# cold-deuu/Quadrotor_Manipulator_MPPI

Hardware: AMD Instinct MI355X
Metric: MPPI rollouts/sec (K x H state-steps) + control-step p50 latency, K=4096 H=32 (higher is better)
Workload: dtype f32

## Files before the change

### quadrotor_manipulator_mppi_amd/csrc/mppi_finalize.hip

```cpp
#include <algorithm>

#include "mppi_device.h"

using namespace mppi;

constexpr int kFinThreads = 512;
constexpr int kMaxRec = 4096;
#ifndef MPPI_FIN_KO
#define MPPI_FIN_KO 0
#endif
#ifndef MPPI_FIN_NOMARK
#define MPPI_FIN_NOMARK 0
#endif
#ifndef MPPI_FIN_XCDS
#define MPPI_FIN_XCDS 8
#endif

#if defined(MPPI_STAMPS) && !defined(MPPI_TIMELINE)
#define FSTAMP(i)                                                                    \
    do {                                                                             \
        __builtin_amdgcn_sched_barrier(0);                                           \
        if (pk.stamps && threadIdx.x == 0)                                           \
            pk.stamps[(((size_t)v * A + a) * ts + sl) * kStamps + (i)] =               \
                __builtin_amdgcn_s_memtime();                                        \
        __builtin_amdgcn_sched_barrier(0);                                           \
    } while (0)
#define FSTAMPRT(i) do { } while (0)
#elif defined(MPPI_STAMPS)
#define FSTAMPRT(i)                                                                  \
    do {                                                                             \
        if (pk.stamps && threadIdx.x == 0) {                                         \
            pk.stamps[(((size_t)v * A + a) * ts + sl) * kStamps + (i)] =               \
                __builtin_amdgcn_s_memrealtime();                                    \
            if ((i) == 13)                                                           \
                pk.stamps[(((size_t)v * A + a) * ts + sl) * kStamps + 15] =            \
                    (unsigned long long)__builtin_amdgcn_s_getreg(0xF814);           \
        }                                                                            \
    } while (0)
#define FSTAMP(i) do { if ((i) == 1 || (i) == 7) FSTAMPRT(i); } while (0)
#else
#define FSTAMP(i) do { } while (0)
#define FSTAMPRT(i) do { } while (0)
#endif

enum { kRoleAny = 0, kRoleFinal = 1, kRoleQuiet = 2, kRolePack = 3, kRolePeer = 4 };
struct GeoRt { static constexpr bool kStatic = false; static constexpr int A = 0, H = 0, tsz = 0, hf = 0, ts = 0; };
template <int A_, int H_, int TSZ_, int HF_, int TS_>
struct GeoC { static constexpr bool kStatic = true; static constexpr int A = A_, H = H_, tsz = TSZ_, hf = HF_, ts = TS_; };

template <int CW, int WIN, int NT, int ROLE, typename GEO>
__device__ __forceinline__ void fin_body(const float* __restrict__ hdr_base, const float* __restrict__ dat_base,
                                         const FinTail* __restrict__ tail, const uint32_t nrec_H, const uint32_t geo,
                                         const int32_t hdr_rs, const int32_t d_rs, const int32_t d_as,
                                         const int32_t hdr_vs, const int32_t d_vs, const uint32_t seq_arg,
                                         const FinParams& pk) {
    constexpr bool kAny = ROLE == kRoleAny, kQuiet = ROLE == kRoleQuiet;
    constexpr bool kOut = kAny || ROLE == kRoleFinal || ROLE == kRolePeer;
    constexpr bool kUpd = kOut || kQuiet;
    constexpr bool kPeer = kAny || ROLE == kRolePeer;
    constexpr int NWV = NT / 64;
    constexpr int ROWS = 64 / CW;
    constexpr int TR = NWV * ROWS;
    constexpr int kNPT = 16;
    __shared__ float wcol[NWV][CW];
    __shared__ float wrho[NWV], wnan[NWV], weta[NWV], weta2[NWV];
    __shared__ float wsg[96];
    const FinParams& p = pk;
    const int tid = threadIdx.x, lane = tid & 63, wv = tid >> 6;
    const int n = (int)(nrec_H & 0xFFFFu);
    const int H = GEO::kStatic ? GEO::H : (int)(nrec_H >> 16);
    const int tsz = GEO::kStatic ? GEO::tsz : (int)(geo & 0xFFu), hf = GEO::kStatic ? GEO::hf : (int)((geo >> 8) & 0xFFu);
    const int ts = GEO::kStatic ? GEO::ts : (int)((geo >> 16) & 0xFFu), A = GEO::kStatic ? GEO::A : (int)(geo >> 24);
    const int x8 = blockIdx.x & 7, j8 = blockIdx.x >> 3, na = (A + MPPI_FIN_XCDS - 1) / MPPI_FIN_XCDS;
    const int sl = (na == 1) ? j8 : (na == 2) ? (j8 >> 1) : j8 / na;
    const int a = x8 + MPPI_FIN_XCDS * (j8 - sl * na), v = blockIdx.y;
    if (x8 >= MPPI_FIN_XCDS || a >= A) return;
    if (MPPI_FIN_KO & 16) { if (tid == 0) p.u_prev[blockIdx.x] = 0.0f; return; }
    FSTAMPRT(13);
    FSTAMP(0);
    const int t_lo = sl * tsz, t_hi = min(H, t_lo + tsz);
    const int w0 = max(0, t_lo - hf), w1 = min(H, t_hi + hf), W = w1 - w0;
    const float* hdr = uniform_ptr(hdr_base + (size_t)v * (uint32_t)hdr_vs);
    const float* col = uniform_ptr(dat_base + (size_t)v * (uint32_t)d_vs + (size_t)a * d_as + w0);
    const FinTail& T = *tail;
    const int g = lane / CW, q = lane - g * CW, gr = wv * ROWS + g;
    const bool qv = q < W;
    float u_old = 0.0f, x0f = 0.0f, v0f = 0.0f;
    double x0d = 0.0, v0d = 0.0;
    float* up = nullptr;

    float coef = 0.0f, dt = 0.0f, dt2 = 0.0f;
    int32_t mode = (ROLE == kRolePack) ? 1 : 0, model = 0, qoff = 0, nq = 0, sf64 = 0, odim = 0;
    const uint32_t seq = seq_arg;
    uint32_t seqv = seq;
    float *wraw = nullptr, *wsmooth = nullptr, *u0p = nullptr, *stats = nullptr;
    double* outp = nullptr;
    uint32_t* flags = nullptr;
    const VehicleConst* vcb = nullptr;
    unsigned long long* const* xpeers = nullptr;
    unsigned long long xpl = 0ull;
    unsigned long long* xlocal = nullptr;
    uint32_t* xovl = nullptr;
    uint32_t* xstall = nullptr;
    unsigned long long* xdec = nullptr;
    int32_t xn = 0, xme = 0;
    uint32_t xstep = 0u, xep = 0u;
    float sg[WIN > 0 ? WIN : 1];
    auto pin_tail = [&]() {
        coef = T.coef;
        if constexpr (kAny) {
            dt = T.dt; dt2 = T.dt2;
            mode = T.mode; model = T.model; qoff = T.qoff; nq = T.nq; sf64 = T.state_f64; odim = T.out_dim;
            wraw = T.wraw; wsmooth = T.wsmooth; u0p = T.u0; stats = T.stats; outp = T.out; flags = T.flags;
            up = T.u_prev; vcb = T.vc;
            xpeers = T.xpeers; xlocal = T.xlocal; xn = T.xn; xme = T.xme; xovl = T.xovl; xstall = T.xstall; xdec = T.xdec;
        } else {
            if constexpr (kOut) {
                dt = T.dt; dt2 = T.dt2;
                model = T.model; qoff = T.qoff; nq = T.nq; sf64 = T.state_f64; odim = T.out_dim;
                u0p = T.u0; stats = T.stats; outp = T.out; flags = T.flags; vcb = T.vc;
            }
            if constexpr (kUpd) up = T.u_prev;
            if constexpr (ROLE == kRolePeer) {
                xpeers = T.xpeers; xlocal = T.xlocal; xn = T.xn; xme = T.xme; xstall = T.xstall; xdec = T.xdec;
            }
        }
        if constexpr (WIN > 0 && kUpd) {
#pragma unroll
            for (int j = 0; j < WIN; ++j) sg[j] = T.sg[j];
        }
        if constexpr (kAny)
            asm volatile("" : "+s"(coef), "+s"(dt), "+s"(dt2), "+s"(mode), "+s"(model), "+s"(qoff), "+s"(nq),
                              "+s"(sf64), "+s"(odim), "+s"(wraw), "+s"(wsmooth), "+s"(u0p), "+s"(stats),
                              "+s"(outp), "+s"(flags), "+s"(up), "+s"(vcb), "+s"(xpeers), "+s"(xlocal), "+s"(xn),
                              "+s"(xme), "+s"(xovl), "+s"(xstall), "+s"(xdec));
        else if constexpr (kOut) {
            asm volatile("" : "+s"(coef), "+s"(dt), "+s"(dt2), "+s"(model), "+s"(qoff), "+s"(nq), "+s"(sf64),
                              "+s"(odim), "+s"(u0p), "+s"(stats), "+s"(outp), "+s"(flags), "+s"(up), "+s"(vcb));
            if constexpr (ROLE == kRolePeer)
                asm volatile("" : "+s"(xpeers), "+s"(xlocal), "+s"(xn), "+s"(xme), "+s"(xstall), "+s"(xdec));
        } else if constexpr (kQuiet)
            asm volatile("" : "+s"(coef), "+s"(up));
        else
            asm volatile("" : "+s"(coef));
        if constexpr (WIN == 9 && kUpd)
            asm volatile("" : "+s"(sg[0]), "+s"(sg[1]), "+s"(sg[2]), "+s"(sg[3]), "+s"(sg[4]), "+s"(sg[5]),
                              "+s"(sg[6]), "+s"(sg[7]), "+s"(sg[8]));
        else if constexpr (WIN == 5 && kUpd)
            asm volatile("" : "+s"(sg[0]), "+s"(sg[1]), "+s"(sg[2]), "+s"(sg[3]), "+s"(sg[4]));
        if constexpr (kUpd) {
            up += (size_t)v * H * A;
            if (wv == 0 && q < W && g == 0) u_old = ld_dev(up + (w0 + q) * A + a);
        }
        if constexpr (kOut) {
            if (tid == 0 && sl == 0) {
                const VehicleConst* vcp = vcb + v;
                x0f = ld_dev(vcp->pos0f + a); v0f = ld_dev(vcp->vel0f + a);
                x0d = ld_dev(vcp->pos0 + a); v0d = ld_dev(vcp->vel0 + a);
                if (seq == kSeqFromVc) seqv = ld_dev((const uint32_t*)vcp->_pad);
            }
        }
        if constexpr (kPeer) {
            if (tid == 0 && xpeers) {
                xstep = ld_dev((const uint32_t*)(vcb + v) + kVcStepWord);
                xep = ld_dev((const uint32_t*)(vcb + v) + kVcEpochWord);
            }
            if (wv == 0 && xpeers)
                xpl = ((const __attribute__((address_space(1))) unsigned long long*)xpeers)[lane < xn ? lane : 0];
        }
    };
    float rho_t = INFINITY, acc = 0.0f, nanflag = 0.0f, eta = 0.0f, eta2 = 0.0f;
    const uint32_t hrs_b = (uint32_t)hdr_rs * 4u, drs_b = (uint32_t)d_rs * 4u;
    const __amdgpu_buffer_rsrc_t hrsrc =
        __builtin_amdgcn_make_buffer_rsrc(const_cast<float*>(hdr), 0, __builtin_amdgcn_readfirstlane((int)((uint32_t)n * hrs_b)),
                                          0x00020000);
    const __amdgpu_buffer_rsrc_t crsrc = __builtin_amdgcn_make_buffer_rsrc(
        const_cast<float*>(col), 0, __builtin_amdgcn_readfirstlane((int)((uint32_t)(n - 1) * drs_b + (uint32_t)W * 4u)),
        0x00020000);
    typedef uint32_t u32x4 __attribute__((ext_vector_type(4)));
    for (int base = 0; base < n; base += TR * kNPT) {
        float4 hd[kNPT];
        float xv[kNPT];
        uint32_t okm = 0;
        const uint32_t r0 = (uint32_t)(base + gr);
        const uint32_t hoff = r0 * hrs_b, coff = r0 * drs_b + (uint32_t)(qv ? q : 0) * 4u;
#pragma unroll
        for (int i = 0; i < kNPT; ++i) {
            okm |= (uint32_t)(r0 + (uint32_t)(i * TR) < (uint32_t)n) << i;
            const u32x4 h = __builtin_amdgcn_raw_buffer_load_b128(hrsrc, (int)(hoff + (uint32_t)(i * TR) * hrs_b), 0, kAuxDev);
            hd[i] = make_float4(__uint_as_float(h.x), __uint_as_float(h.y), __uint_as_float(h.z), __uint_as_float(h.w));
            xv[i] = __uint_as_float(__builtin_amdgcn_raw_buffer_load_b32(crsrc, (int)(coff + (uint32_t)(i * TR) * drs_b), 0, kAuxDev));
        }
        if (base == 0) {
            __builtin_amdgcn_sched_barrier(0);
            pin_tail();
        }
#pragma unroll
        for (int i = 0; i < kNPT; ++i)
            if (!((okm >> i) & 1u)) hd[i].x = INFINITY;
        FSTAMP(7);
        float m = INFINITY;
#pragma unroll
        for (int i = 0; i < kNPT; ++i) { m = fminf(m, hd[i].x); nanflag = fmaxf(nanflag, hd[i].w); }
        float fr[kNPT];
#pragma unroll
        for (int i = 0; i < kNPT; ++i) fr[i] = 0.0f;
        if (m < INFINITY) {
            const float rn = fminf(rho_t, m);
            if (rho_t < INFINITY) {
                const float sc = __expf(coef * (rho_t - rn));
                acc *= sc;
                eta *= sc;
                eta2 *= sc * sc;
            }
            rho_t = rn;
#pragma unroll
            for (int i = 0; i < kNPT; ++i) {
                const float f = (hd[i].x < INFINITY) ? __expf(coef * (hd[i].x - rn)) : 0.0f;
                fr[i] = f;
                eta = fmaf(f, hd[i].y, eta);
                eta2 = fmaf(f * f, hd[i].z, eta2);
            }
        }
#pragma unroll
        for (int i = 0; i < kNPT; ++i) acc = fmaf(fr[i], xv[i], acc);
        FSTAMP(8);
    }
    {
        const float rw = fold_rows<CW>(rho_t, OpMin());
        const float sc = (rho_t < INFINITY) ? __expf(coef * (rho_t - rw)) : 0.0f;
        acc = fold_rows<CW>(acc * sc, OpAdd());
        const float e1 = fold_rows<CW>(eta * sc, OpAdd()), e2 = fold_rows<CW>(eta2 * (sc * sc), OpAdd());
        const float nf = fold_rows<CW>(nanflag, OpMax());
        if (lane < CW) wcol[wv][lane] = acc;
        if (lane == 0) { wrho[wv] = rw; wnan[wv] = nf; weta[wv] = e1; weta2[wv] = e2; }
    }
    FSTAMP(1);
    if (MPPI_FIN_KO & 8) { if (lane < CW) p.u_prev[lane] += acc + (float)eta; return; }
    lds_barrier();
    if (wv != 0) return;
    FSTAMP(2);
    float rho = wrho[0], nanf = wnan[0];
#pragma unroll
    for (int w = 1; w < NWV; ++w) { rho = fminf(rho, wrho[w]); nanf = fmaxf(nanf, wnan[w]); }
    float N = 0.0f;
    eta = 0.0f; eta2 = 0.0f;
#pragma unroll
    for (int w = 0; w < NWV; ++w) {
        const float f = (wrho[w] < INFINITY) ? __expf(coef * (wrho[w] - rho)) : 0.0f;
        N = fmaf(f, (lane < CW) ? wcol[w][lane] : 0.0f, N);
        eta = fmaf(f, weta[w], eta);
        eta2 = fmaf(f * f, weta2[w], eta2);
    }
    FSTAMP(3);
    bool xlate = false;
    if (kPeer && xpeers != nullptr && mode != 1) {
        const uint32_t step = __builtin_amdgcn_readfirstlane(xstep);
        const uint32_t tag = peer_tag(step, __builtin_amdgcn_readfirstlane(xep));
        const size_t nbk = (size_t)8 * na * ts, blk = blockIdx.x;
        const size_t par = step & 1u;
        const float hown = (lane == 0) ? rho : (lane == 1) ? eta : (lane == 2) ? eta2 : nanf;
        const size_t off = ((par * (size_t)xn + (size_t)xme) * nbk + blk) * kXW;
        typedef __attribute__((address_space(1))) unsigned long long gst64;
        auto region = [&](int d) {
            return (gst64*)(((uint64_t)(uint32_t)__builtin_amdgcn_readlane((int)(uint32_t)(xpl >> 32), d) << 32) |
                            (uint32_t)__builtin_amdgcn_readlane((int)(uint32_t)xpl, d));
        };
        typedef __attribute__((address_space(1))) unsigned long long gu64;
        gu64* const ctl = (gu64*)xlocal - kXCtl;
        if (mode == 0) {
            if (uint32_t* xs = xstall) {
                const uint32_t sv = ld_dev(xs);
                if (sv != 0u && (sv & 0xFFFFu) == (uint32_t)blk) {
                    const uint64_t t_s = __builtin_amdgcn_s_memrealtime(), ticks = (uint64_t)(sv >> 16) * 100000ull;
                    while (__builtin_amdgcn_s_memrealtime() - t_s < ticks) __builtin_amdgcn_s_sleep(127);
                    if (lane == 0) __hip_atomic_store(xs, 0u, __ATOMIC_RELAXED, __HIP_MEMORY_SCOPE_AGENT);
                }
            }
            const unsigned long long wc = ((unsigned long long)tag << 32) | __float_as_uint(N);
            const unsigned long long wh = ((unsigned long long)tag << 32) | __float_as_uint(hown);
#pragma unroll
            for (int d = 0; d < kMaxPeers; ++d) {
                if (d >= xn || d == xme) continue;
                gst64* dst = region(d) + off;
                if (lane < W) __hip_atomic_store(dst + kHdr + lane, wc, __ATOMIC_RELAXED, __HIP_MEMORY_SCOPE_SYSTEM);
                if (lane < kHdr) __hip_atomic_store(dst + lane, wh, __ATOMIC_RELAXED, __HIP_MEMORY_SCOPE_SYSTEM);
            }
        }
        float nv[kMaxPeers], hv[kMaxPeers];
#pragma unroll
        for (int r = 0; r < kMaxPeers; ++r) {
            nv[r] = (r == xme) ? N : 0.0f;
            hv[r] = (r == xme) ? hown : 0.0f;
        }
        const bool needc = lane < W, needh = lane < kHdr;
        uint32_t pend = ((1u << xn) - 1u) & ~(1u << xme);
        const unsigned long long* src = xlocal + (par * (size_t)xn * nbk + blk) * kXW;
        auto poll = [&](bool heed_reports) -> bool {
            const uint64_t t_in = __builtin_amdgcn_s_memrealtime();
            while (pend != 0u) {
                unsigned long long xc[kMaxPeers], xh[kMaxPeers];
#pragma unroll
                for (int r = 0; r < kMaxPeers; ++r) {
                    xc[r] = 0ull; xh[r] = 0ull;
                    if ((pend >> r) & 1u) {
                        gu64* s = (gu64*)(src + (size_t)r * nbk * kXW);
                        xc[r] = __hip_atomic_load(s + kHdr + lane, __ATOMIC_RELAXED, __HIP_MEMORY_SCOPE_SYSTEM);
                        xh[r] = __hip_atomic_load(s + (lane & (kHdr - 1)), __ATOMIC_RELAXED, __HIP_MEMORY_SCOPE_SYSTEM);
                    }
                }
                if (heed_reports) {
                    const unsigned long long xk = __hip_atomic_load(ctl + (lane < xn ? lane : 0), __ATOMIC_RELAXED,
                                                                    __HIP_MEMORY_SCOPE_SYSTEM);
                    if (__builtin_amdgcn_ballot_w64(lane < xn && xk != 0ull) != 0ull) return true;
                }
#pragma unroll
                for (int r = 0; r < kMaxPeers; ++r) {
                    if (!((pend >> r) & 1u)) continue;
                    const bool ok = (!needc || (uint32_t)(xc[r] >> 32) == tag) && (!needh || (uint32_t)(xh[r] >> 32) == tag);
                    if (__builtin_amdgcn_ballot_w64(!ok) == 0ull) {
                        nv[r] = needc ? __uint_as_float((uint32_t)xc[r]) : 0.0f;
                        hv[r] = needh ? __uint_as_float((uint32_t)xh[r]) : 0.0f;
                        pend &= ~(1u << r);
                    }
                }
                pend = __builtin_amdgcn_readfirstlane(pend);
                if (pend == 0u) break;
                if (__builtin_amdgcn_s_memrealtime() - t_in > kPeerWaitTicks) return true;
                __builtin_amdgcn_s_sleep(1);
            }
            return false;
        };
        bool late = poll(true), torn = false;
        if (mode == 0) {
            gu64* dw = (gu64*)xdec + par * nbk;
            if (!late) {
                if (lane == 0 && !MPPI_FIN_NOMARK)
                    __hip_atomic_store(dw + blk, ((unsigned long long)tag << 32) | kDecCommit, __ATOMIC_RELAXED,
                                       __HIP_MEMORY_SCOPE_AGENT);
            } else {
                const unsigned long long cw = ((unsigned long long)tag << 32) | 1ull;
#pragma unroll
                for (int d = 0; d < kMaxPeers; ++d) {
                    if (d >= xn) continue;
                    gst64* rg = region(d);
                    if (lane == 0) __hip_atomic_store(rg - kXCtl + xme, cw, __ATOMIC_RELAXED, __HIP_MEMORY_SCOPE_SYSTEM);
                }
                const uint64_t t_rep = __builtin_amdgcn_s_memrealtime();
                while (__builtin_amdgcn_s_memrealtime() - t_rep < kDecGraceTicks) __builtin_amdgcn_s_sleep(8);
                bool marked = false;
                for (size_t i = lane; i < nbk; i += 64) {
                    const unsigned long long w = __hip_atomic_load(dw + i, __ATOMIC_RELAXED, __HIP_MEMORY_SCOPE_AGENT);
                    marked |= (uint32_t)(w >> 32) == tag && ((uint32_t)w & 3u) == kDecCommit;
                }
                if (__builtin_amdgcn_ballot_w64(marked) != 0ull) {
                    late = poll(false);
                    torn = late;
                }
                uint32_t* xe = T.xerr;
                if (late && lane == 0 && xe) {
                    __hip_atomic_store(xe, tag, __ATOMIC_RELAXED, __HIP_MEMORY_SCOPE_SYSTEM);
                    if (torn) __hip_atomic_store(xe + 1, tag, __ATOMIC_RELAXED, __HIP_MEMORY_SCOPE_SYSTEM);
                }
            }
        }
        rho = INFINITY;
        nanf = late ? (torn ? 3.0f : 2.0f) : 0.0f;
#pragma unroll
        for (int r = 0; r < kMaxPeers; ++r) {
            if (r < xn) {
                rho = fminf(rho, __int_as_float(__builtin_amdgcn_readlane(__float_as_int(hv[r]), 0)));
                nanf = fmaxf(nanf, __int_as_float(__builtin_amdgcn_readlane(__float_as_int(hv[r]), 3)));
            }
        }
        N = 0.0f; eta = 0.0f; eta2 = 0.0f;
#pragma unroll
        for (int r = 0; r < kMaxPeers; ++r) {
            if (r < xn) {
                const float rr = __int_as_float(__builtin_amdgcn_readlane(__float_as_int(hv[r]), 0));
                const float er = __int_as_float(__builtin_amdgcn_readlane(__float_as_int(hv[r]), 1));
                const float e2 = __int_as_float(__builtin_amdgcn_readlane(__float_as_int(hv[r]), 2));
                const float f = (rr < INFINITY) ? __expf(coef * (rr - rho)) : 0.0f;
                N = fmaf(f, nv[r], N);
                eta = fmaf(f, er, eta);
                eta2 = fmaf(f * f, e2, eta2);
            }
        }
        if (late) { xlate = true; N = 0.0f; }
    }
    const int t = w0 + lane;
    const bool own = lane < W && t >= t_lo && t < t_hi;
    if (mode == 1) {
        float* dst = T.dst;
        float* xbase = T.xbase;
        int64_t xslot = T.xslot;
        int32_t nslots = T.nslots, myslot = T.myslot, P = T.P;
        asm volatile("" : "+s"(dst), "+s"(xbase), "+s"(xslot), "+s"(nslots), "+s"(myslot), "+s"(P));
        dst += (size_t)v * P;
        if (a == 0 && sl == 0 && lane == 0) {
            dst[0] = rho; dst[1] = eta; dst[2] = eta2; dst[3] = nanf;
        }
        if (own) dst[kHdr + a * H + t] = N;
        for (int s = 0; s < nslots; ++s) {
            if (s == myslot) continue;
            float* z = xbase + (size_t)s * xslot + (size_t)v * P;
            if (a == 0 && sl == 0 && lane < kHdr) z[lane] = 0.0f;
            if (own) z[kHdr + a * H + t] = 0.0f;
        }
        FSTAMPRT(14);
        return;
    }

    const float etaf = xlate ? 1.0f : (nanf > 0.0f) ? NAN : eta;
    const float w = __fdividef(N, etaf);
    FSTAMP(4);
    constexpr int kPad = kMaxW / 2;
    static_assert(kPad + 64 + kMaxW / 2 <= (int)(sizeof(wsg) / sizeof(float)),
                  "wsg holds the widest window: kPad + W (<= 64) + hf");
    float sm = 0.0f;
    if (lane < W) {
        wsg[kPad + lane] = w;
        if (w0 == 0 && t < hf) wsg[kPad - 1 - t] = w;
        if (w1 == H && t >= H - hf) wsg[kPad + 2 * H - 1 - t - w0] = w;
    }
    wave_lds_handoff();
    {
        const float* src = wsg + kPad + lane - hf;
        if constexpr (WIN > 0) {
#pragma unroll
            for (int j = 0; j < WIN; ++j) sm = fmaf(sg[j], src[j], sm);
        } else {
            for (int j = 0; j < T.window; ++j) sm = fmaf(T.sg[j], src[j], sm);
        }
    }
// ... 18 lines not shown
        if (plain) u0p[(size_t)v * A + a] = u0;
        double* out = outp + (size_t)v * odim;
        const bool drone_dim = (model == MPPI_MODEL_DRONE) || (model == MPPI_MODEL_WHOLEBODY && a < 3);
        double o1 = 0.0, o2 = 0.0;
        if (model == MPPI_MODEL_QUADROTOR) {
        } else if (drone_dim) {
            const float x0 = x0f, v0 = v0f;
            const float xo = (x0 + v0 * dt) + (0.5f * u0) * dt2;
            const float vo = v0 + dt * u0;
            o1 = xo;
            o2 = vo;
            if (plain) {
                out[a] = o1;
                out[3 + a] = o2;
            }
        } else {
            const int j = a - qoff;
            const int base = (model == MPPI_MODEL_WHOLEBODY) ? 6 : 0;
            const float t1 = uold0 * dt;
            const float t2 = ((0.5f * u0) * dt) * dt;
            const float t3 = u0 * dt;
            if (sf64 && model == MPPI_MODEL_ARM) {
                o1 = (x0d + (double)t1) + (double)t2;
                o2 = v0d + (double)t3;
            } else {
                o1 = (double)((x0f + t1) + t2);
                o2 = (double)(v0f + t3);
            }
            if (plain) {
                out[base + j] = o1;
                out[base + nq + j] = o2;
            }
        }
        const float ess = (eta2 > 0.0f) ? eta * (eta / eta2) : 0.0f;
        if (plain && a == 0) {
            float* st = stats + (size_t)v * 4;
            st[0] = rho;
            st[1] = eta;
            st[2] = ess;
            st[3] = nanf;
        }
        if (seqv != 0u) {
            typedef uint32_t u32x4 __attribute__((ext_vector_type(4)));
            u32x4* rec = reinterpret_cast<u32x4*>(flags) + (size_t)v * (2 * A + 1);
            const uint64_t b1 = (uint64_t)__double_as_longlong(o1), b2 = (uint64_t)__double_as_longlong(o2);
            rec[2 * a] = u32x4{(uint32_t)b1, (uint32_t)(b1 >> 32), __float_as_uint(u0), seqv};
            rec[2 * a + 1] = u32x4{(uint32_t)b2, (uint32_t)(b2 >> 32), __float_as_uint(nanf), seqv};
            if (a == 0) rec[2 * A] = u32x4{__float_as_uint(rho), __float_as_uint(eta), __float_as_uint(ess), seqv};
        }
    }
    FSTAMP(6);
    FSTAMPRT(14);
    if (!(MPPI_FIN_KO & 128)) asm volatile("s_waitcnt vmcnt(0)" ::: "memory");
    if (xovl != nullptr && mode == 0 && lane == 0)
        __hip_atomic_fetch_add(xovl + ((size_t)v * A + a) * ts + sl, 1u, __ATOMIC_RELAXED, __HIP_MEMORY_SCOPE_AGENT);
}

template <int CW, int WIN, int NT>
__global__ void __launch_bounds__(NT) k_finalize(const float* __restrict__ hdr_base,
                                                          const float* __restrict__ dat_base,
                                                          const FinTail* __restrict__ tail,
                                                          const uint32_t nrec_H, const uint32_t geo,
                                                          const int32_t hdr_rs, const int32_t d_rs,
                                                          const int32_t d_as, const int32_t hdr_vs,
                                                          const int32_t d_vs, const uint32_t seq_arg,
                                                          const FinParams pk) {
    fin_body<CW, WIN, NT, kRoleAny, GeoRt>(hdr_base, dat_base, tail, nrec_H, geo, hdr_rs, d_rs, d_as, hdr_vs, d_vs,
                                           seq_arg, pk);
}

template <int GID> struct FinGeo;
template <> struct FinGeo<1> { typedef GeoC<7, 32, 8, 4, 4> type; static constexpr int win = 9; };
template <> struct FinGeo<2> { typedef GeoC<3, 32, 8, 2, 4> type; static constexpr int win = 5; };
template <> struct FinGeo<3> { typedef GeoC<4, 32, 8, 2, 4> type; static constexpr int win = 5; };
template <> struct FinGeo<4> { typedef GeoC<10, 64, 8, 4, 8> type; static constexpr int win = 9; };
constexpr int kFinGeoCW = 16;
static int fin_geo_id(const FinParams* p) {
    if (p->tsz != 8 || p->half != p->window / 2 || p->ts * 8 != p->H) return 0;
    if (p->window == 9) return (p->H == 32 && p->A == 7) ? 1 : (p->H == 64 && p->A == 10) ? 4 : 0;
    if (p->window == 5) return (p->H == 32 && p->A == 3) ? 2 : (p->H == 32 && p->A == 4) ? 3 : 0;
    return 0;
}

template <int NT, int ROLE, int GID>
__global__ void __launch_bounds__(NT) k_finalize_s(const float* __restrict__ hdr_base,
                                                            const float* __restrict__ dat_base,
                                                            const FinTail* __restrict__ tail,
                                                            const uint32_t nrec_H, const uint32_t geo,
                                                            const int32_t hdr_rs, const int32_t d_rs,
                                                            const int32_t d_as, const int32_t hdr_vs,
                                                            const int32_t d_vs, const uint32_t seq_arg,
                                                            const FinParams pk) {
    fin_body<kFinGeoCW, FinGeo<GID>::win, NT, ROLE, typename FinGeo<GID>::type>(hdr_base, dat_base, tail, nrec_H, geo, hdr_rs,
                                                                          d_rs, d_as, hdr_vs, d_vs, seq_arg, pk);
}

extern "C" __global__ void __launch_bounds__(64) k_dispatch_probe(unsigned long long* out) {
    if (threadIdx.x == 0) out[0] = mppi_dispatch_id();
}

extern "C" __global__ void __launch_bounds__(64) k_peer_probe(unsigned long long* const* peers,
                                                              unsigned long long* local, int n, int me,
                                                              unsigned long long slot_words, uint32_t tag,
                                                              unsigned long long ticks,
                                                              unsigned long long* out) {
    const int lane = threadIdx.x;
    const unsigned long long w = ((unsigned long long)(tag | (uint32_t)me) << 32) | 0x3F800000ull;
    if (lane < n) __hip_atomic_store(peers[lane] + (size_t)me * slot_words, w, __ATOMIC_RELAXED, __HIP_MEMORY_SCOPE_SYSTEM);
    unsigned long long got = 0ull;
    if (lane < n) {
        const uint64_t t0 = __builtin_amdgcn_s_memrealtime();
        for (;;) {
            got = __hip_atomic_load(local + (size_t)lane * slot_words, __ATOMIC_RELAXED, __HIP_MEMORY_SCOPE_SYSTEM);
            if ((uint32_t)(got >> 32) == (tag | (uint32_t)lane)) break;
            if (__builtin_amdgcn_s_memrealtime() - t0 > ticks) break;
            __builtin_amdgcn_s_sleep(2);
        }
        out[lane] = got;
    }
}

extern "C" int mppi_launch_peer_probe(unsigned long long* const* peers, unsigned long long* local, int n, int me,
                                      unsigned long long slot_words, uint32_t tag, unsigned long long ticks,
                                      unsigned long long* out, void* stream) {
    hipLaunchKernelGGL(k_peer_probe, dim3(1), dim3(64), 0, (hipStream_t)stream, peers, local, n, me, slot_words, tag,
                       ticks, out);
    return (int)hipGetLastError();
}

__global__ void k_weights(const float* S, const float* stats, float* w, int V, int K, float coef) {
    const int i = blockIdx.x * blockDim.x + threadIdx.x;
    if (i >= V * K) return;
    const int v = i / K;
    const float rho = stats[v * 4], eta = stats[v * 4 + 1];
    w[i] = expf(coef * (S[i] - rho)) / eta;
}

extern "C" int mppi_launch_finalize(const FinParams* p, void* stream) {
    const int W = std::min(p->H, p->tsz + 2 * p->half);
    if (p->nrec > kMaxRec || p->nrec <= 0 || p->H > MPPI_MAX_HORIZON || p->tsz > 255 || p->half > 255 ||
        p->ts > 255 || p->A > 255 || W > 64 || !p->tail || p->hdr_vs > 0x7fffffff || p->d_vs > 0x7fffffff)
        return -1;
    const uint32_t nh = (uint32_t)p->nrec | ((uint32_t)p->H << 16);
    const uint32_t geo = (uint32_t)p->tsz | ((uint32_t)p->half << 8) | ((uint32_t)p->ts << 16) | ((uint32_t)p->A << 24);
    const int cw = (W <= 16) ? 16 : (W <= 32) ? 32 : 64;
    int nt = 512;
    for (int c : {128, 256})
        if (c * 16 / cw >= p->nrec) { nt = c; break; }
    const dim3 grid(8 * ((p->A + MPPI_FIN_XCDS - 1) / MPPI_FIN_XCDS) * p->ts, p->V), block(nt);
    hipStream_t s = (hipStream_t)stream;
    const int gid = ((p->kern & kFinKernGeneric) || p->xovl) ? 0 : fin_geo_id(p);
    const int role = !gid ? kRoleAny
                     : p->mode == 1 ? kRolePack
                     : p->mode != 0 ? kRoleAny
                     : p->xpeers ? kRolePeer
                     : (p->kern & kFinKernQuiet) ? kRoleQuiet : kRoleFinal;
#define MPPI_FIN_SGO(NTV, ROLEV, GIDV)                                                                    \
    return go(k_finalize_s<NTV, ROLEV, GIDV>,                                                             \
              [](char* b, size_t n) {                                                                     \
                  snprintf(b, n, "_Z12k_finalize_sILi%dELi%dELi%dEEvPKfS1_PKN4mppi7FinTailEjjiiiiijNS2_9FinParamsE", \
                           NTV, ROLEV, GIDV);                                                             \
              },                                                                                          \
              grid, block, 0, s, p->hdr, p->dat, p->tail, nh, geo, (int32_t)p->hdr_rs, (int32_t)p->d_rs,   \
              (int32_t)p->d_as, (int32_t)p->hdr_vs, (int32_t)p->d_vs, p->seq, *p)
#define MPPI_FIN_SNT(ROLEV, GIDV)                                                                         \
    do {                                                                                                  \
        if (nt == 128) MPPI_FIN_SGO(128, ROLEV, GIDV);                                                    \
        else if (nt == 256) MPPI_FIN_SGO(256, ROLEV, GIDV);                                               \
        else MPPI_FIN_SGO(512, ROLEV, GIDV);                                                              \
    } while (0)
#define MPPI_FIN_SGEO(ROLEV)                                                                              \
    do {                                                                                                  \
        if (gid == 1) MPPI_FIN_SNT(ROLEV, 1);                                                             \
        else if (gid == 2) MPPI_FIN_SNT(ROLEV, 2);                                                        \
        else if (gid == 3) MPPI_FIN_SNT(ROLEV, 3);                                                        \
        else MPPI_FIN_SNT(ROLEV, 4);                                                                      \
    } while (0)
    if (role == kRoleFinal) MPPI_FIN_SGEO(kRoleFinal);
    else if (role == kRoleQuiet) MPPI_FIN_SGEO(kRoleQuiet);
    else if (role == kRolePack) MPPI_FIN_SGEO(kRolePack);
    else if (role == kRolePeer) MPPI_FIN_SGEO(kRolePeer);
#undef MPPI_FIN_SGEO
#undef MPPI_FIN_SNT
#undef MPPI_FIN_SGO
#define MPPI_FIN_GO(CWV, WINV, NTV)                                                                      \
    return go(k_finalize<CWV, WINV, NTV>,                                                                 \
              [](char* b, size_t n) {                                                                     \
                  snprintf(b, n, "_Z10k_finalizeILi%dELi%dELi%dEEvPKfS1_PKN4mppi7FinTailEjjiiiiijNS2_9FinParamsE", \
                           CWV, WINV, NTV);                                                               \
              },                                                                                          \
              grid, block, 0, s, p->hdr, p->dat, p->tail, nh, geo, (int32_t)p->hdr_rs, (int32_t)p->d_rs,   \
              (int32_t)p->d_as, (int32_t)p->hdr_vs, (int32_t)p->d_vs, p->seq, *p)
#define MPPI_FIN_LAUNCH(CWV, WINV)                                                                        \
    do {                                                                                                  \
        if (nt == 128) MPPI_FIN_GO(CWV, WINV, 128);                                                       \
        else if (nt == 256) MPPI_FIN_GO(CWV, WINV, 256);                                                  \
        else MPPI_FIN_GO(CWV, WINV, 512);                                                                 \
    } while (0)
#define MPPI_FIN_WIN(CWV)                                                                                 \
    do {                                                                                                  \
        if (p->window == 9) MPPI_FIN_LAUNCH(CWV, 9);                                                      \
        else if (p->window == 5) MPPI_FIN_LAUNCH(CWV, 5);                                                 \
        else MPPI_FIN_LAUNCH(CWV, 0);                                                                     \
    } while (0)
    if (W <= 16) MPPI_FIN_WIN(16);
    else if (W <= 32) MPPI_FIN_WIN(32);
    else MPPI_FIN_WIN(64);
#undef MPPI_FIN_WIN
#undef MPPI_FIN_LAUNCH
#undef MPPI_FIN_GO
    return -1;
}

#ifdef MPPI_PROBE
__global__ void __launch_bounds__(256) k_boundary(float* scratch) {
    if (blockIdx.x == 0 && threadIdx.x == 0) scratch[0] = 0.0f;
}
extern "C" int mppi_launch_boundary(float* scratch, int blocks, void* stream) {
    hipLaunchKernelGGL(k_boundary, dim3(blocks), dim3(256), 0, (hipStream_t)stream, scratch);
    return (int)hipGetLastError();
}
#endif

extern "C" int mppi_launch_weights(const float* S, const float* stats, float* w, int V, int K, float coef,
                                   void* stream) {
    const int n = V * K;
    hipLaunchKernelGGL(k_weights, dim3((n + 255) / 256), dim3(256), 0, (hipStream_t)stream, S, stats, w, V,
                       K, coef);
    return (int)hipGetLastError();
}
```

### quadrotor_manipulator_mppi_amd/csrc/mppi_step.cpp

```cpp
#include <emmintrin.h>

#include <algorithm>
#include <atomic>
#include <chrono>
#include <cmath>
#include <cstddef>
#include <cstdio>
#include <cstdlib>
#include <cstring>
#include <string>
#include <vector>

#include "mppi_engine.h"

using namespace mppi;

namespace mppi_host {

void block_records(const mppi_engine* e, FinParams& f) {
    const int64_t nb = e->dp.nb, H = e->H;
    f.nrec = (int32_t)nb;
    f.hdr = e->d_hdr; f.hdr_vs = nb * 4; f.hdr_rs = 4;
    f.dat = e->d_rdata; f.d_vs = (int64_t)e->A * nb * H; f.d_as = nb * H; f.d_rs = H;
}

void final_records(const mppi_engine* e, FinParams& f) {
    if (sharded(e)) {
        const int64_t P = e->dp.P;
        f.nrec = e->cfg.shard_count;
        f.hdr = e->d_exchange; f.hdr_vs = P; f.hdr_rs = (int64_t)e->V * P;
        f.dat = e->d_exchange + kHdr; f.d_vs = P; f.d_as = e->H; f.d_rs = (int64_t)e->V * P;
    } else {
        block_records(e, f);
    }
}

}

using namespace mppi_host;

static bool quiet_steps(const mppi_engine* e) {
    return !(e->generic & 3) && !e->timing && !e->d_stamps && !e->d_fstamps && !e->out_dbg && !e->no_flag_dbg && !e->overlap;
}

static bool quiet_rollout(const mppi_engine* e) {
    return quiet_steps(e) && !(e->generic & 8) && !e->peer && !sharded(e);
}

static mppi_status rollout_impl(mppi_engine* e, const float* d_noise, bool quiet) {
    if (!e) return fail(MPPI_ERR_INVALID_ARG, "null engine");
    if (!e->state_set) return fail(MPPI_ERR_STATE, "mppi_rollout before mppi_set_state");
    if (e->cfg.noise_mode == MPPI_NOISE_INJECTED && !d_noise)
        return fail(MPPI_ERR_INVALID_ARG, "INJECTED noise mode needs a device noise buffer");
    if (sharded(e) && !e->d_exchange)
        return fail(MPPI_ERR_STATE, "shard_count > 1 needs mppi_bind_exchange or mppi_comm_init");
    if (use_device(e)) return MPPI_ERR_HIP;
    DevParams p = e->dp;
    p.noise_in = d_noise;
    p.vc0 = e->h_vc[0];
    p.step_ctr = e->step_ctr;
    if (quiet && quiet_rollout(e)) p.kern |= kRollKernQuiet;
    hipEvent_t e0 = nullptr, e1 = nullptr;
    if (e->timing) { e0 = pool_event(e); e1 = pool_event(e); HIP_TRY(hipEventRecord(e0, e->stream)); }
    int rc = mppi_launch_rollout(&p, e->threads, e->stream);
    if (rc != 0) return fail(MPPI_ERR_HIP, "rollout launch failed (%d: %s)", rc,
                             rc > 0 ? hipGetErrorString((hipError_t)rc) : "no kernel for this model/A/H");
    if (e->timing) {
        HIP_TRY(hipEventRecord(e1, e->stream));
        e->roll_pairs.emplace_back(e0, e1);
        if (e->roll_pairs.size() >= 2048) { mppi_status st = drain_timing(e); if (st) return st; }
    }
    if (sharded(e)) {
        FinParams f = e->fp;
        pack_fields(e, f);
        f.tail = e->d_tail + kTailPack;
        if (f.stamps) f.stamps += (size_t)e->V * e->A * e->fin_ts * kStamps;
        block_records(e, f);
        rc = mppi_launch_finalize(&f, e->stream);
        if (rc != 0) return fail(MPPI_ERR_HIP, "pack launch failed (%d)", rc);
    }
    return MPPI_OK;
}

extern "C" {

mppi_status mppi_rollout(mppi_engine* e, const float* d_noise) { return rollout_impl(e, d_noise, false); }

static std::string fin_symbol(const FinParams& f) {
    LaunchDesc d{};
    mppi_aql::set_capture(&d);
    const int rc = mppi_launch_finalize(&f, nullptr);
    mppi_aql::set_capture(nullptr);
    return rc == 0 ? d.symbol : "?";
}
static std::string roll_symbol(const DevParams& p, int threads) {
    LaunchDesc d{};
    mppi_aql::set_capture(&d);
    const int rc = mppi_launch_rollout(&p, threads, nullptr);
    mppi_aql::set_capture(nullptr);
    return rc == 0 ? d.symbol : "?";
}
static std::string kernels_text(const std::string& roll, const std::string& fin, const std::string* quiet,
                                const std::string* roll_quiet = nullptr) {
    std::string s = "rollout " + roll + ", finalize " + fin;
    if (quiet) s += ", quiet finalize " + (*quiet == fin ? std::string("none") : *quiet);
    if (roll_quiet) s += ", quiet rollout " + (*roll_quiet == roll ? std::string("none") : *roll_quiet);
    return s;
}

static mppi_status finalize_impl(mppi_engine* e, bool record_out, bool quiet = false) {
    if (use_device(e)) return MPPI_ERR_HIP;
    FinParams f = e->fp;
    f.mode = 0;
    if (quiet && !record_out && quiet_steps(e)) f.kern |= kFinKernQuiet;
    f.seq = 0u;
    if (record_out && !e->no_flag_dbg) {
        f.seq = ++e->seq_ctr & 0x7FFFFFFFu;
        if (f.seq == 0u) f.seq = ++e->seq_ctr & 0x7FFFFFFFu;
    }
    final_records(e, f);
    if (e->out_dbg == 1 && !record_out) f.tail = e->d_tail + kTailScratch;
    hipEvent_t e0 = nullptr, e1 = nullptr;
    if (e->timing) { e0 = pool_event(e); e1 = pool_event(e); HIP_TRY(hipEventRecord(e0, e->stream)); }
    int rc = mppi_launch_finalize(&f, e->stream);
    if (rc != 0) return fail(MPPI_ERR_HIP, "finalize launch failed (%d)", rc);
    if (e->timing) { HIP_TRY(hipEventRecord(e1, e->stream)); e->fin_pairs.emplace_back(e0, e1); }
    if (record_out) e->out_seq = f.seq;
    if (record_out) HIP_TRY(hipEventRecord(e->ev_out, e->stream));
    ++e->step_ctr;
    e->out_pending = record_out;
    e->aql_out = false;
    e->aql_call = false;
    return MPPI_OK;
}

mppi_status mppi_finalize(mppi_engine* e) {
    if (!e) return fail(MPPI_ERR_INVALID_ARG, "null engine");
    return finalize_impl(e, true);
}

static bool records_tagged(const mppi_engine* e, uint32_t want) {
    const volatile uint32_t* r = (const volatile uint32_t*)(e->h_out + off_flags(e));
    const size_t n = rec_count(e);
    for (size_t i = 0; i < n; ++i)
        if (r[4 * i + 3] != want) return false;
    return true;
}

static inline bool load_record(const mppi_engine* e, size_t i, uint32_t want, uint32_t (&w)[4]) {
    const __m128i x = _mm_load_si128((const __m128i*)(e->h_out + off_flags(e)) + i);
    _mm_storeu_si128((__m128i*)w, x);
    return w[3] == want;
}

static mppi_status wait_outputs(mppi_engine* e) {
    if (e->aql_out) return aql_join(e);
    if (e->aql_call) {
        const uint32_t want = e->out_seq;
        const auto t0 = std::chrono::steady_clock::now();
        for (uint64_t it = 1;; ++it) {
            if (records_tagged(e, want)) break;
            if ((it & 255u) == 0) {
                if (const int q = mppi_aql::step_error(e->aql)) return fail(MPPI_ERR_HIP, "native queue error %d", q);
                if (std::chrono::steady_clock::now() - t0 > std::chrono::seconds(60))
                    return fail(MPPI_ERR_HIP, "native control call: no outputs after 60 s");
            }
            __builtin_ia32_pause();
        }
        std::atomic_thread_fence(std::memory_order_acquire);
        mppi_aql::step_call_read(e->aql);
        e->call_wait_us = std::chrono::duration<double, std::micro>(std::chrono::steady_clock::now() - t0).count();
        return MPPI_OK;
    }
    if (!e->event_wait) {
        const uint32_t want = e->out_seq;
// ... 363 lines not shown
        if (rc != 0) return fail(MPPI_ERR_HIP, "describing the step's launches failed (%d)", rc);
        e->call_p = p;
        e->call_f = f;
        e->call_threads = e->threads;
        e->call_cached = true;
    }
    if (prof) {
        const auto q4 = std::chrono::steady_clock::now();
        const std::chrono::steady_clock::time_point qs[5] = {q0, q1, q2, q3, q4};
        for (int i = 0; i < 4; ++i) pacc[i] += std::chrono::duration<double, std::micro>(qs[i + 1] - qs[i]).count();
        if (++pcn % 1000 == 0)
            fprintf(stderr, "[mppi aql] call setup (us): hipSetDevice %.2f  vehicle constants %.2f  stream query %.2f  "
                            "capture %.2f\n", pacc[0] / pcn, pacc[1] / pcn, pacc[2] / pcn, pacc[3] / pcn);
    }
    const uint32_t seq_off = roll.arg_bytes - (uint32_t)sizeof(DevParams) + (uint32_t)offsetof(DevParams, vc0) +
                             (uint32_t)offsetof(VehicleConst, _pad);
    std::string err;
    uint32_t seq = 0;
    const int pr = mppi_aql::step_call(e->aql, roll, fin, e->step_ctr, kRollStepOff, seq_off, &seq, &err);
    if (pr == -2) {
        e->aql_off = true;
        e->aql_why = err;
        return e->aql_mode == 1 ? fail(MPPI_ERR_STATE, "native dispatch: %s", err.c_str()) : MPPI_OK;
    }
    if (pr != 0) return fail(MPPI_ERR_HIP, "native dispatch: %s", err.c_str());
    ++e->step_ctr;
    e->out_seq = seq;
    e->out_pending = true;
    e->aql_out = false;
    e->aql_call = true;
    if (!hit || e->kern_call_hip) e->kern_call = kernels_text(roll.symbol, fin.symbol, nullptr);
    e->kern_call_hip = false;
    *used = true;
    return MPPI_OK;
}

mppi_status mppi_run_steps(mppi_engine* e, int32_t n) {
    if (!e || n < 0) return fail(MPPI_ERR_INVALID_ARG, "mppi_run_steps: bad arguments");
    if (sharded(e) && !e->comm) return fail(MPPI_ERR_STATE, "mppi_run_steps on a shard needs mppi_comm_init");
    if (e->cfg.noise_mode != MPPI_NOISE_PHILOX) return fail(MPPI_ERR_STATE, "mppi_run_steps needs device noise");
    if (!e->state_set) return fail(MPPI_ERR_STATE, "mppi_run_steps before mppi_set_state");
    if (n == 0) return MPPI_OK;
    bool used = false;
    mppi_status st = run_steps_aql(e, n, &used);
    if (st != MPPI_OK || used) return st;
    for (int i = 0; i < n; ++i) {
        mppi_status st = rollout_impl(e, nullptr, i < n - 1);
        if (st != MPPI_OK) return st;
        if (e->comm && (st = mppi_exchange(e)) != MPPI_OK) return st;
        if ((st = finalize_impl(e, i == n - 1, true)) != MPPI_OK) return st;
    }
    {
        DevParams p = e->dp;
        p.vc0 = e->h_vc[0];
        FinParams f = e->fp;
        f.mode = 0;
        final_records(e, f);
        const std::string full = fin_symbol(f);
        if (n > 1 && quiet_steps(e)) f.kern |= kFinKernQuiet;
        const std::string q = fin_symbol(f), roll = roll_symbol(p, e->threads);
        if (n > 1 && quiet_rollout(e)) p.kern |= kRollKernQuiet;
        const std::string rq = roll_symbol(p, e->threads);
        e->kern_batch = kernels_text(roll, full, &q, &rq);
        e->kern_batch_state = 0;
    }
    return MPPI_OK;
}

mppi_status mppi_kernel_info(mppi_engine* e, char* buf, int32_t len) {
    if (!e || !buf || len <= 0) return fail(MPPI_ERR_INVALID_ARG, "mppi_kernel_info: bad arguments");
    snprintf(buf, (size_t)len, "batch: %s; call: %s%s", e->kern_batch.c_str(), e->kern_call.c_str(),
             e->generic == kGenericAll ? "; MPPI_GENERIC_KERNELS" : e->generic ? "; MPPI_GENERIC_KERNELS (in part)" : "");
    return MPPI_OK;
}

mppi_status mppi_dispatch_info(mppi_engine* e, char* buf, int32_t len) {
    if (!e || !buf || len <= 0) return fail(MPPI_ERR_INVALID_ARG, "mppi_dispatch_info: bad arguments");
    snprintf(buf, (size_t)len, "%s%s; calls: %s%s%s", e->aql_why.empty() ? "aql" : "hip: ", e->aql_why.c_str(),
             e->calls_native ? "aql (arguments in " : "hip", e->calls_native ? mppi_aql::step_call_memory(e->aql) : "",
             e->calls_native ? ")" : "");
    return MPPI_OK;
}

int32_t mppi_debug_finalize_kernels(const int32_t* g, char* full, char* quiet, int32_t len) {
    if (!g || !full || !quiet || len <= 0) return MPPI_ERR_INVALID_ARG;
    static const FinTail tail{};
    static unsigned long long* const peers[1] = {nullptr};
    FinParams f;
    std::memset(&f, 0, sizeof(f));
    f.V = 1; f.A = g[0]; f.H = g[1]; f.tsz = g[2]; f.half = g[3]; f.ts = g[4]; f.window = g[5]; f.nrec = g[6];
    f.mode = g[7];
    f.tail = &tail;
    if (g[8]) f.xpeers = peers;
    f.kern = g[9] ? kFinKernGeneric : 0;
    const std::string a = fin_symbol(f);
    if (!g[9]) f.kern |= kFinKernQuiet;
    const std::string b = fin_symbol(f);
    snprintf(full, (size_t)len, "%s", a.c_str());
    snprintf(quiet, (size_t)len, "%s", b.c_str());
    return (a == "?" || b == "?") ? MPPI_ERR_INVALID_ARG : MPPI_OK;
}

int32_t mppi_debug_rollout_kernels(const int32_t* g, char* full, char* quiet, int32_t len) {
    if (!g || !full || !quiet || len <= 0) return MPPI_ERR_INVALID_ARG;
    DevParams p;
    std::memset(&p, 0, sizeof(p));
    p.model = g[0]; p.A = g[1]; p.H = g[2]; p.L = g[3]; p.nch = g[4]; p.iters = g[5]; p.V = g[7];
    p.R = p.L > 0 ? 64 / p.L : 0;
    p.state_f64 = g[8]; p.noise_mode = g[9]; p.store_noise = g[10]; p.cost_terms = g[11]; p.sigma_diag = !g[12];
    p.nb = 16; p.K = 16; p.store_traj = 1;
    p.chain_fast = 2;
    p.kern = g[14] ? kRollKernGeneric : 0;
    const std::string a = roll_symbol(p, g[6]);
    if (!g[13] && !g[14]) p.kern |= kRollKernQuiet;
    const std::string b = roll_symbol(p, g[6]);
    snprintf(full, (size_t)len, "%s", a.c_str());
    snprintf(quiet, (size_t)len, "%s", b.c_str());
    return (a == "?" || b == "?") ? MPPI_ERR_INVALID_ARG : MPPI_OK;
}

mppi_status mppi_synchronize(mppi_engine* e) {
    if (!e) return fail(MPPI_ERR_INVALID_ARG, "null engine");
    if (use_device(e)) return MPPI_ERR_HIP;
    if (e->out_pending && !e->event_wait && !e->aql_out) {
        mppi_status st = wait_outputs(e);
        if (st != MPPI_OK) return st;
    }
    HIP_TRY(hipStreamSynchronize(e->stream));
    if (e->peer)
        if (const uint32_t t = sticky_timeout(e))
            return fail(MPPI_ERR_PEER_TIMEOUT, "peer exchange: a step was given up (tag %08x): this rank's "
                                               "warm start may differ from its peers' until mppi_peer_reset", t);
    return MPPI_OK;
}

int32_t mppi_debug_queue_touch(mppi_engine* e) {
    if (!e || !e->aql) return MPPI_ERR_INVALID_ARG;
    std::string err;
    const int r = mppi_aql::step_touch(e->aql, false, &err);
    return r == 0 ? MPPI_OK : fail(MPPI_ERR_HIP, "queue touch: %s", err.c_str());
}


int64_t mppi_debug_stamps(mppi_engine* e, unsigned long long* out, int64_t max_waves) {
    if (!e || !out) return MPPI_ERR_INVALID_ARG;
    if (!e->d_stamps) return 0;
    if (use_device(e)) return MPPI_ERR_HIP;
    const int64_t nwaves = std::min<int64_t>(max_waves, (int64_t)e->V * e->dp.nb * (e->threads / 64));
    if (hipStreamSynchronize(e->stream) != hipSuccess ||
        hipMemcpy(out, e->d_stamps, (size_t)nwaves * kStamps * 8, hipMemcpyDeviceToHost) != hipSuccess)
        return MPPI_ERR_HIP;
    return nwaves;
}

int64_t mppi_debug_fstamps(mppi_engine* e, unsigned long long* out, int64_t max_blocks, int32_t which) {
    if (!e || !out || which < 0 || which > 1) return MPPI_ERR_INVALID_ARG;
    if (!e->d_fstamps) return 0;
    if (use_device(e)) return MPPI_ERR_HIP;
    const int64_t nb = (int64_t)e->V * e->A * e->fin_ts;
    const int64_t n = std::min<int64_t>(max_blocks, nb);
    if (hipStreamSynchronize(e->stream) != hipSuccess ||
        hipMemcpy(out, e->d_fstamps + (size_t)which * nb * kStamps, (size_t)n * kStamps * 8, hipMemcpyDeviceToHost) !=
            hipSuccess)
        return MPPI_ERR_HIP;
    return n;
}

int32_t mppi_debug_queue_ring(mppi_engine* e) {
    if (!e || !e->aql) return MPPI_ERR_INVALID_ARG;
    if (e->pw_us.load()) return fail(MPPI_ERR_STATE, "mppi_debug_queue_ring: the prewarm thread also writes packets");
    mppi_aql::step_ring(e->aql);
    return MPPI_OK;
}

}
```

Before: 17.14 billion.

## Process multiple columns per lane in finalize kernel with vector loads

The specialized finalize kernel now has each lane handle CPL (default 4) consecutive time columns. It loads them with b64/b128 buffer loads and keeps per-column accumulators, so blocks launch with NT/CPL threads. The cross-row reduction becomes a DPP plus permlane16_swap fold, and a single-wave block uses a wave-level LDS handoff instead of a block barrier. This is meant to cut thread count, barrier cost and load instruction count on a latency-bound reduction, at the cost of more per-lane work, a realignment offset, and new lane mapping logic that carries correctness risk.

Measured after the change: 17.79 billion (median of 6 runs). 1.04x the previous value.

```diff
diff --git a/quadrotor_manipulator_mppi_amd/csrc/mppi_finalize.hip b/quadrotor_manipulator_mppi_amd/csrc/mppi_finalize.hip
--- a/quadrotor_manipulator_mppi_amd/csrc/mppi_finalize.hip
+++ b/quadrotor_manipulator_mppi_amd/csrc/mppi_finalize.hip
@@ -48,7 +48,7 @@
 template <int A_, int H_, int TSZ_, int HF_, int TS_>
 struct GeoC { static constexpr bool kStatic = true; static constexpr int A = A_, H = H_, tsz = TSZ_, hf = HF_, ts = TS_; };
 
-template <int CW, int WIN, int NT, int ROLE, typename GEO>
+template <int CW, int WIN, int NT, int ROLE, typename GEO, int CPL = 1>
 __device__ __forceinline__ void fin_body(const float* __restrict__ hdr_base, const float* __restrict__ dat_base,
                                          const FinTail* __restrict__ tail, const uint32_t nrec_H, const uint32_t geo,
                                          const int32_t hdr_rs, const int32_t d_rs, const int32_t d_as,
@@ -62,6 +62,9 @@
     constexpr int ROWS = 64 / CW;
     constexpr int TR = NWV * ROWS;
     constexpr int kNPT = 16;
+    static_assert(CPL == 1 || ((CPL == 2 || CPL == 4) && CW == 16 && NT / CPL >= 32), "lane maps: see above");
+    constexpr int LPR = CW / CPL;
+    constexpr int kLanes = NT / CPL < 64 ? NT / CPL : 64;
     __shared__ float wcol[NWV][CW];
     __shared__ float wrho[NWV], wnan[NWV], weta[NWV], weta2[NWV];
     __shared__ float wsg[96];
@@ -81,10 +84,14 @@
     const int t_lo = sl * tsz, t_hi = min(H, t_lo + tsz);
     const int w0 = max(0, t_lo - hf), w1 = min(H, t_hi + hf), W = w1 - w0;
     const float* hdr = uniform_ptr(hdr_base + (size_t)v * (uint32_t)hdr_vs);
-    const float* col = uniform_ptr(dat_base + (size_t)v * (uint32_t)d_vs + (size_t)a * d_as + w0);
+    const int doff = CPL == 1 ? 0 : w0 & (CPL - 1);
+    const float* col = uniform_ptr(dat_base + (size_t)v * (uint32_t)d_vs + (size_t)a * d_as + (CPL == 1 ? w0 : w0 - doff));
     const FinTail& T = *tail;
-    const int g = lane / CW, q = lane - g * CW, gr = wv * ROWS + g;
-    const bool qv = q < W;
+    const int g = CPL == 1 ? lane / CW : (lane >> 3) & 3, q = CPL == 1 ? lane - g * CW : lane & (LPR - 1);
+    const int wo = CPL == 1 ? wv : CPL == 4 ? wv * 4 + (((lane >> 2) & 1) | ((lane >> 5) << 1)) : wv * 2 + (lane >> 5);
+    const int gr = wo * ROWS + g;
+    const int nqd = (doff + W + CPL - 1) / CPL;
+    const bool qv = CPL == 1 ? q < W : q < nqd;
     float u_old = 0.0f, x0f = 0.0f, v0f = 0.0f;
     double x0d = 0.0, v0d = 0.0;
     float* up = nullptr;
@@ -150,7 +157,11 @@
             asm volatile("" : "+s"(sg[0]), "+s"(sg[1]), "+s"(sg[2]), "+s"(sg[3]), "+s"(sg[4]));
         if constexpr (kUpd) {
             up += (size_t)v * H * A;
-            if (wv == 0 && q < W && g == 0) u_old = ld_dev(up + (w0 + q) * A + a);
+            if constexpr (CPL == 1) {
+                if (wv == 0 && q < W && g == 0) u_old = ld_dev(up + (w0 + q) * A + a);
+            } else {
+                if (wv == 0 && lane < W) u_old = ld_dev(up + (w0 + lane) * A + a);
+            }
         }
         if constexpr (kOut) {
             if (tid == 0 && sl == 0) {
@@ -169,27 +180,42 @@
                 xpl = ((const __attribute__((address_space(1))) unsigned long long*)xpeers)[lane < xn ? lane : 0];
         }
     };
-    float rho_t = INFINITY, acc = 0.0f, nanflag = 0.0f, eta = 0.0f, eta2 = 0.0f;
+    float rho_t = INFINITY, nanflag = 0.0f, eta = 0.0f, eta2 = 0.0f;
+    float acc[CPL];
+#pragma unroll
+    for (int j = 0; j < CPL; ++j) acc[j] = 0.0f;
     const uint32_t hrs_b = (uint32_t)hdr_rs * 4u, drs_b = (uint32_t)d_rs * 4u;
     const __amdgpu_buffer_rsrc_t hrsrc =
         __builtin_amdgcn_make_buffer_rsrc(const_cast<float*>(hdr), 0, __builtin_amdgcn_readfirstlane((int)((uint32_t)n * hrs_b)),
                                           0x00020000);
     const __amdgpu_buffer_rsrc_t crsrc = __builtin_amdgcn_make_buffer_rsrc(
-        const_cast<float*>(col), 0, __builtin_amdgcn_readfirstlane((int)((uint32_t)(n - 1) * drs_b + (uint32_t)W * 4u)),
+        const_cast<float*>(col), 0,
+        __builtin_amdgcn_readfirstlane((int)((uint32_t)(n - 1) * drs_b + (uint32_t)(CPL == 1 ? W : nqd * CPL) * 4u)),
         0x00020000);
     typedef uint32_t u32x4 __attribute__((ext_vector_type(4)));
+    typedef uint32_t u32x2 __attribute__((ext_vector_type(2)));
     for (int base = 0; base < n; base += TR * kNPT) {
         float4 hd[kNPT];
-        float xv[kNPT];
+        float xv[kNPT][CPL];
         uint32_t okm = 0;
         const uint32_t r0 = (uint32_t)(base + gr);
-        const uint32_t hoff = r0 * hrs_b, coff = r0 * drs_b + (uint32_t)(qv ? q : 0) * 4u;
+        const uint32_t hoff = r0 * hrs_b, coff = r0 * drs_b + (uint32_t)(qv ? q : 0) * (uint32_t)(4 * CPL);
 #pragma unroll
         for (int i = 0; i < kNPT; ++i) {
             okm |= (uint32_t)(r0 + (uint32_t)(i * TR) < (uint32_t)n) << i;
             const u32x4 h = __builtin_amdgcn_raw_buffer_load_b128(hrsrc, (int)(hoff + (uint32_t)(i * TR) * hrs_b), 0, kAuxDev);
             hd[i] = make_float4(__uint_as_float(h.x), __uint_as_float(h.y), __uint_as_float(h.z), __uint_as_float(h.w));
-            xv[i] = __uint_as_float(__builtin_amdgcn_raw_buffer_load_b32(crsrc, (int)(coff + (uint32_t)(i * TR) * drs_b), 0, kAuxDev));
+            const int bo = (int)(coff + (uint32_t)(i * TR) * drs_b);
+            if constexpr (CPL == 4) {
+                const u32x4 b = __builtin_amdgcn_raw_buffer_load_b128(crsrc, bo, 0, kAuxDev);
+                xv[i][0] = __uint_as_float(b.x); xv[i][1] = __uint_as_float(b.y);
+                xv[i][2] = __uint_as_float(b.z); xv[i][3] = __uint_as_float(b.w);
+            } else if constexpr (CPL == 2) {
+                const u32x2 b = __builtin_amdgcn_raw_buffer_load_b64(crsrc, bo, 0, kAuxDev);
+                xv[i][0] = __uint_as_float(b.x); xv[i][1] = __uint_as_float(b.y);
+            } else {
+                xv[i][0] = __uint_as_float(__builtin_amdgcn_raw_buffer_load_b32(crsrc, bo, 0, kAuxDev));
+            }
         }
         if (base == 0) {
             __builtin_amdgcn_sched_barrier(0);
@@ -209,7 +235,8 @@
             const float rn = fminf(rho_t, m);
             if (rho_t < INFINITY) {
                 const float sc = __expf(coef * (rho_t - rn));
-                acc *= sc;
+#pragma unroll
+                for (int j = 0; j < CPL; ++j) acc[j] *= sc;
                 eta *= sc;
                 eta2 *= sc * sc;
             }
@@ -223,21 +250,46 @@
             }
         }
 #pragma unroll
-        for (int i = 0; i < kNPT; ++i) acc = fmaf(fr[i], xv[i], acc);
+        for (int i = 0; i < kNPT; ++i) {
+#pragma unroll
+            for (int j = 0; j < CPL; ++j) acc[j] = fmaf(fr[i], xv[i][j], acc[j]);
+        }
         FSTAMP(8);
     }
-    {
+    if constexpr (CPL == 1) {
         const float rw = fold_rows<CW>(rho_t, OpMin());
         const float sc = (rho_t < INFINITY) ? __expf(coef * (rho_t - rw)) : 0.0f;
-        acc = fold_rows<CW>(acc * sc, OpAdd());
+        acc[0] = fold_rows<CW>(acc[0] * sc, OpAdd());
         const float e1 = fold_rows<CW>(eta * sc, OpAdd()), e2 = fold_rows<CW>(eta2 * (sc * sc), OpAdd());
         const float nf = fold_rows<CW>(nanflag, OpMax());
-        if (lane < CW) wcol[wv][lane] = acc;
+        if (lane < CW) wcol[wv][lane] = acc[0];
         if (lane == 0) { wrho[wv] = rw; wnan[wv] = nf; weta[wv] = e1; weta2[wv] = e2; }
+    } else {
+        auto fold_g = [](float x, auto op) {
+            asm volatile("" : "+v"(x));
+            x = op(x, dpp_all<0x128>(x));
+            const auto r = __builtin_amdgcn_permlane16_swap(__float_as_uint(x), __float_as_uint(x), false, false);
+            return op(__uint_as_float(r[0]), __uint_as_float(r[1]));
+        };
+        const float rw = fold_g(rho_t, OpMin());
+        const float sc = (rho_t < INFINITY) ? __expf(coef * (rho_t - rw)) : 0.0f;
+#pragma unroll
+        for (int j = 0; j < CPL; ++j) acc[j] = fold_g(acc[j] * sc, OpAdd());
+        const float e1 = fold_g(eta * sc, OpAdd()), e2 = fold_g(eta2 * (sc * sc), OpAdd());
+        const float nf = fold_g(nanflag, OpMax());
+        if (g == 0) {
+#pragma unroll
+            for (int j = 0; j < CPL; ++j) {
+                const int wq = q * CPL + j - doff;
+                if (wq >= 0 && wq < W) wcol[wo][wq] = acc[j];
+            }
+            if (q == 0) { wrho[wo] = rw; wnan[wo] = nf; weta[wo] = e1; weta2[wo] = e2; }
+        }
     }
     FSTAMP(1);
-    if (MPPI_FIN_KO & 8) { if (lane < CW) p.u_prev[lane] += acc + (float)eta; return; }
-    lds_barrier();
+    if (MPPI_FIN_KO & 8) { if (lane < CW) p.u_prev[lane] += acc[0] + (float)eta; return; }
+    if constexpr (NT / CPL <= 64) wave_lds_handoff();
+    else lds_barrier();
     if (wv != 0) return;
     FSTAMP(2);
     float rho = wrho[0], nanf = wnan[0];
@@ -349,7 +401,7 @@
                 const uint64_t t_rep = __builtin_amdgcn_s_memrealtime();
                 while (__builtin_amdgcn_s_memrealtime() - t_rep < kDecGraceTicks) __builtin_amdgcn_s_sleep(8);
                 bool marked = false;
-                for (size_t i = lane; i < nbk; i += 64) {
+                for (size_t i = lane; i < nbk; i += kLanes) {
                     const unsigned long long w = __hip_atomic_load(dw + i, __ATOMIC_RELAXED, __HIP_MEMORY_SCOPE_AGENT);
                     marked |= (uint32_t)(w >> 32) == tag && ((uint32_t)w & 3u) == kDecCommit;
                 }
@@ -534,8 +586,12 @@
     return 0;
 }
 
+#ifndef MPPI_FIN_CPL
+#define MPPI_FIN_CPL 4
+#endif
+constexpr int kFinCPL = MPPI_FIN_CPL;
 template <int NT, int ROLE, int GID>
-__global__ void __launch_bounds__(NT) k_finalize_s(const float* __restrict__ hdr_base,
+__global__ void __launch_bounds__(NT / kFinCPL) k_finalize_s(const float* __restrict__ hdr_base,
                                                             const float* __restrict__ dat_base,
                                                             const FinTail* __restrict__ tail,
                                                             const uint32_t nrec_H, const uint32_t geo,
@@ -543,7 +599,7 @@
                                                             const int32_t d_as, const int32_t hdr_vs,
                                                             const int32_t d_vs, const uint32_t seq_arg,
                                                             const FinParams pk) {
-    fin_body<kFinGeoCW, FinGeo<GID>::win, NT, ROLE, typename FinGeo<GID>::type>(hdr_base, dat_base, tail, nrec_H, geo, hdr_rs,
+    fin_body<kFinGeoCW, FinGeo<GID>::win, NT, ROLE, typename FinGeo<GID>::type, kFinCPL>(hdr_base, dat_base, tail, nrec_H, geo, hdr_rs,
                                                                           d_rs, d_as, hdr_vs, d_vs, seq_arg, pk);
 }
 
@@ -613,8 +669,8 @@
                   snprintf(b, n, "_Z12k_finalize_sILi%dELi%dELi%dEEvPKfS1_PKN4mppi7FinTailEjjiiiiijNS2_9FinParamsE", \
                            NTV, ROLEV, GIDV);                                                             \
               },                                                                                          \
-              grid, block, 0, s, p->hdr, p->dat, p->tail, nh, geo, (int32_t)p->hdr_rs, (int32_t)p->d_rs,   \
-              (int32_t)p->d_as, (int32_t)p->hdr_vs, (int32_t)p->d_vs, p->seq, *p)
+              grid, dim3(NTV / kFinCPL), 0, s, p->hdr, p->dat, p->tail, nh, geo, (int32_t)p->hdr_rs,       \
+              (int32_t)p->d_rs, (int32_t)p->d_as, (int32_t)p->hdr_vs, (int32_t)p->d_vs, p->seq, *p)
 #define MPPI_FIN_SNT(ROLEV, GIDV)                                                                         \
     do {                                                                                                  \
         if (nt == 128) MPPI_FIN_SGO(128, ROLEV, GIDV);                                                    \
diff --git a/quadrotor_manipulator_mppi_amd/csrc/mppi_step.cpp b/quadrotor_manipulator_mppi_amd/csrc/mppi_step.cpp
--- a/quadrotor_manipulator_mppi_amd/csrc/mppi_step.cpp
+++ b/quadrotor_manipulator_mppi_amd/csrc/mppi_step.cpp
@@ -86,11 +86,12 @@
 
 mppi_status mppi_rollout(mppi_engine* e, const float* d_noise) { return rollout_impl(e, d_noise, false); }
 
-static std::string fin_symbol(const FinParams& f) {
+static std::string fin_symbol(const FinParams& f, LaunchDesc* desc = nullptr) {
     LaunchDesc d{};
     mppi_aql::set_capture(&d);
     const int rc = mppi_launch_finalize(&f, nullptr);
     mppi_aql::set_capture(nullptr);
+    if (desc) *desc = d;
     return rc == 0 ? d.symbol : "?";
 }
 static std::string roll_symbol(const DevParams& p, int threads) {
@@ -620,6 +621,7 @@
     return MPPI_OK;
 }
 
+static thread_local int32_t g_fin_launch[6];
 int32_t mppi_debug_finalize_kernels(const int32_t* g, char* full, char* quiet, int32_t len) {
     if (!g || !full || !quiet || len <= 0) return MPPI_ERR_INVALID_ARG;
     static const FinTail tail{};
@@ -631,12 +633,23 @@
     f.tail = &tail;
     if (g[8]) f.xpeers = peers;
     f.kern = g[9] ? kFinKernGeneric : 0;
-    const std::string a = fin_symbol(f);
+    LaunchDesc da{}, db{};
+    const std::string a = fin_symbol(f, &da);
     if (!g[9]) f.kern |= kFinKernQuiet;
-    const std::string b = fin_symbol(f);
+    const std::string b = fin_symbol(f, &db);
     snprintf(full, (size_t)len, "%s", a.c_str());
     snprintf(quiet, (size_t)len, "%s", b.c_str());
+    const LaunchDesc* ds[2] = {&da, &db};
+    for (int i = 0; i < 2; ++i) {
+        g_fin_launch[3 * i] = (int32_t)ds[i]->block[0];
+        g_fin_launch[3 * i + 1] = (int32_t)ds[i]->grid[0];
+        g_fin_launch[3 * i + 2] = (int32_t)ds[i]->lds;
+    }
     return (a == "?" || b == "?") ? MPPI_ERR_INVALID_ARG : MPPI_OK;
+}
+
+void mppi_debug_finalize_launch(int32_t* out6) {
+    if (out6) std::memcpy(out6, g_fin_launch, sizeof(g_fin_launch));
 }
 
 int32_t mppi_debug_rollout_kernels(const int32_t* g, char* full, char* quiet, int32_t len) {
```
